# Aster32/GAN-DANet

Hardware: AMD Instinct MI355X
Metric: train samples/sec (G+D step) on 256x256 tiles (higher is better)
Workload: dtype bf16; 1 GPU; full G+D train step, 8ch 256x256 -> 1024x1024 tiles, batch 32/GPU (global 32), perceptual=on, SSIM evaluated, AdamW x2; survey_config=3, per_gpu_batch=32, global_batch=32, tile=256, parallelism=dp1

## Files before the change

### gan-danet_amd/_lib.py

```python
from __future__ import annotations

import ctypes as C
import os

HERE = os.path.dirname(os.path.abspath(__file__))
LIB_PATH = os.path.join(HERE, "lib", "libgandanet_hip.so")

PREC_FP32, PREC_BF16, PREC_X3 = 0, 1, 2
PAM_BWD_K64_ATOMIC, PAM_BWD_K64_PARTS, PAM_BWD_K32_PARTS, PAM_BWD_TWO_KERNEL = 0, 1, 2, 3
ACT_NONE, ACT_RELU, ACT_LEAKY02, ACT_SIGMOID = 0, 1, 2, 3
EVAL_F64, EVAL_SKIP_NAN = 1, 2
GUARD_SQNORM, GUARD_NORM, GUARD_COEF, GUARD_OK, GUARD_APPLIED, GUARD_SKIPPED, GUARD_RECORD = range(7)
GUARD_CHUNK = 65536
FILTER_F32, FILTER_F64 = 0, 1
EDGE_REFLECT, EDGE_INTERIOR = 0, 1
FILTER_MAX_RADIUS, SAVGOL_MAX_WINDOW = 64, 33
ZOOM_MIRROR, ZOOM_NEAREST = 0, 1
FREQ_MAX_BINS, FREQ_MAX_TABLE_BYTES = 33, 16 << 20
ZONE_MAX, ZONE_EDGE_CHUNK = 32, 512
STL_MAX_T = 2048
SKILL_MAPS = ("n", "mean_p", "mean_t", "bias", "rmse", "mae", "std_p", "std_t", "cc", "nse", "kge", "crmsd")
LSTSQ_MAX_P = 8
TREND_MAX_T = 2048
TREND_MAPS = ("n", "s", "var_s", "z", "p", "tau", "slope", "intercept", "slope_lo", "slope_hi")
# ... 5 lines not shown
ENSV_M_COVER, ENSV_M_RELIABILITY, ENSV_M_TIED, ENSV_M_HIST, ENSV_METRICS = 6, 10, 11, 12, 45
ENSV_LEVELS = (0.5, 0.6826894921370859, 0.9, 0.95)
EOF_MAX_T, EOF_MAX_K = 256, 16
EOF_CHUNK, EOF_SPLIT_MIN, EOF_SPLIT_MAX = 32, 8, 256

c_fp = C.c_void_p


class ConvDesc(C.Structure):
    _fields_ = [
        ("B", C.c_int), ("M", C.c_int), ("Mstore", C.c_int), ("Ck", C.c_int), ("ks", C.c_int),
        ("stride", C.c_int), ("pad", C.c_int), ("transposed", C.c_int),
        ("Hi", C.c_int), ("Wi", C.c_int), ("Ho", C.c_int), ("Wo", C.c_int),
        ("a", c_fp), ("a_bs", C.c_long), ("a_sm", C.c_long), ("a_sc", C.c_long), ("a_st", C.c_long),
        ("x", c_fp), ("x_bs", C.c_long),
        ("in_scale", c_fp), ("in_shift", c_fp), ("in_relu", C.c_int),
        ("y", c_fp), ("y_bs", C.c_long),
        ("out_layout", C.c_int), ("out_bf16", C.c_int), ("ldo", C.c_int),
        ("alpha", c_fp), ("bias", c_fp), ("res", c_fp), ("res_bs", C.c_long),
        ("act", C.c_int), ("accumulate", C.c_int), ("precision", C.c_int),
        ("sub_oy", C.c_int), ("sub_ox", C.c_int), ("sub_step", C.c_int),
    ]


class GemmNTDesc(C.Structure):
    _fields_ = [
        ("B", C.c_int), ("M", C.c_int), ("N", C.c_int), ("kseg", C.c_int), ("klen", C.c_long),
        ("a", c_fp), ("a_bs", C.c_long), ("a_ss", C.c_long), ("lda", C.c_long),
        ("bm", c_fp), ("b_bs", C.c_long), ("b_ss", C.c_long), ("ldb", C.c_long),
        ("im2col", C.c_int), ("ks", C.c_int), ("stride", C.c_int), ("pad", C.c_int),
        ("Hi", C.c_int), ("Wi", C.c_int), ("Ho", C.c_int), ("Wo", C.c_int),
        ("in_scale", c_fp), ("in_shift", c_fp), ("in_relu", C.c_int),
        ("c", c_fp), ("c_bs", C.c_long), ("ldc", C.c_long),
        ("alpha", c_fp), ("bias", c_fp),
        ("accumulate", C.c_int), ("splits", C.c_int), ("precision", C.c_int),
    ]


_i, _l, _f, _p, _sz = C.c_int, C.c_long, C.c_float, c_fp, C.c_size_t

SIGNATURES = {
    "gd_version": (_i, []),
    "gd_set_deterministic": (None, [_i]),
    "gd_get_deterministic": (_i, []),
    "gd_set_det_reduce": (_i, [_i]),
    "gd_get_det_reduce": (_i, []),
    "gd_last_error": (_i, [C.c_char_p, _i]),
    "gd_sizeof_conv_desc": (_i, []),
    "gd_sizeof_gemm_nt_desc": (_i, []),
    "gd_conv2d": (_i, [C.POINTER(ConvDesc), _p]),
    "gd_gemm_nt": (_i, [C.POINTER(GemmNTDesc), _p]),
    "gd_gemm_nt_ws": (_i, [C.POINTER(GemmNTDesc), _p, _p, _sz]),
    "gd_gemm_nt_plan": (_i, [C.POINTER(GemmNTDesc), _sz, C.POINTER(_i), C.POINTER(_sz)]),
    "gd_conv3x3_ws_bytes": (_sz, [_i, _i]),
    "gd_conv3x3_eligible": (_i, [C.POINTER(ConvDesc)]),
    "gd_conv3x3": (_i, [C.POINTER(ConvDesc), _p, _sz, _p]),
    "gd_conv3x3_wgrad": (_i, [_p, _l, _p, _p, _l, _p, _i, _p, _p, _i, _i, _i, _i, _i, _i, _i, _i, _p, _p]),
    "gd_conv3x3_wgrad_ws": (_i, [_p, _l, _p, _p, _l, _p, _i, _p, _p, _i, _i, _i, _i, _i, _i, _i, _i, _p, _p, _p, _sz]),
    "gd_conv3x3_wgrad_plan": (_i, [_i, _i, _i, _i, _i, _i, _sz, C.POINTER(_i), C.POINTER(_sz)]),
    "gd_pack_16_split": (_i, [_p, _l, _i, _i, _i, _p, _p, _i, _p, _l, _i, _l, _i, _i, _p, _l, _i, _l, _i, _i, _p]),
    "gd_pack_16_split_masked": (_i, [_p, _l, _i, _i, _i, _p, _p, _i, _p, _l, _i, _l, _i, _i, _p, _l, _i, _l, _i, _i, _p, _l, _p]),
    "gd_split3_weights": (_i, [_p, _l, _l, _l, _p, _p]),
    "gd_bn_stats_ws_floats": (_sz, [_i, _i, _l]),
    "gd_bn_stats": (_i, [_p, _l, _i, _i, _l, _f, _f, _p, _p, _p, _p, _p, _p]),
    "gd_bn_fold": (_i, [_p, _p, _p, _p, _i, _p, _p, _p]),
    "gd_bn_fold_eval": (_i, [_p, _p, _p, _p, _f, _i, _p, _p, _p, _p]),
    "gd_affine_act": (_i, [_p, _l, _p, _p, _i, _i, _l, _i, _p, _l, _p]),
    "gd_bn_act_bwd": (_i, [_p, _l, _p, _l, _p, _p, _p, _p, _p, _i, _i, _l, _i, _i, _p, _p, _p, _l, _i, _p, _p]),
    "gd_bn_stats_local": (_i, [_p, _l, _i, _i, _l, _p, _p, _p]),
    "gd_bn_stats_merge": (_i, [_p, _i, _i, _f, _f, _p, _p, _p, _p, _p]),
    "gd_bn_act_bwd_dx": (_i, [_p, _l, _p, _l, _p, _p, _p, _p, _p, _p, _f, _i, _i, _l, _i, _p, _l, _i, _p]),
    "gd_bicubic_fwd": (_i, [_p, _i, _i, _i, _p, _i, _i, _f, _f, _p]),
    "gd_bicubic_bwd": (_i, [_p, _i, _i, _i, _p, _i, _i, _f, _f, _p]),
    "gd_bilinear_fwd": (_i, [_p, _i, _i, _i, _p, _i, _i, _i, _p, _p]),
    "gd_bilinear_bwd": (_i, [_p, _i, _i, _i, _p, _i, _i, _p]),
    "gd_maxpool2_fwd": (_i, [_p, _i, _i, _i, _p, _p]),
    "gd_maxpool2_bwd": (_i, [_p, _p, _i, _i, _i, _p, _p]),
    "gd_act_fwd": (_i, [_p, _p, _l, _i, _p]),
    "gd_act_bwd": (_i, [_p, _p, _p, _l, _i, _p]),
    "gd_axpby": (_i, [_p, _f, _p, _f, _l, _p]),
    "gd_scale_dev": (_i, [_p, _p, _p, _l, _i, _p]),
    "gd_copy_rows": (_i, [_p, _l, _l, _p, _l, _l, _i, _i, _i, _p]),
    "gd_channel_sum": (_i, [_p, _l, _i, _i, _l, _p, _i, _p, _p]),
    "gd_copy_slab": (_i, [_p, _l, _p, _l, _i, _l, _i, _p]),
    "gd_softmax_rows": (_i, [_p, _p, _l, _i, _f, _p]),
    "gd_softmax_rows_bwd": (_i, [_p, _p, _p, _l, _i, _f, _p]),
    "gd_dot": (_i, [_p, _p, _l, _p, _i, _p, _p]),
    "gd_transpose": (_i, [_p, _p, _i, _i, _i, _p]),
    "gd_add_transpose": (_i, [_p, _p, _i, _i, _p]),
    "gd_bce_logits": (_i, [_p, _l, _f, _p, _p, _p, _p]),
    "gd_bce_logits_target": (_i, [_p, _p, _l, _p, _p, _p, _p, _p]),
    "gd_leaky_fwd": (_i, [_p, _p, _l, _f, _p]),
    "gd_leaky_bwd": (_i, [_p, _p, _p, _l, _f, _p]),
    "gd_mse": (_i, [_p, _p, _l, _p, _p, _p, _p]),
    "gd_l1": (_i, [_p, _p, _l, _p, _p, _p, _p]),
    "gd_tv": (_i, [_p, _i, _i, _i, _i, _f, _p, _p, _p, _p]),
    "gd_ssim": (_i, [_p, _p, _i, _i, _i, _i, _p, _p, _p]),
    "gd_ssim_samples": (_i, [_p, _p, _i, _i, _i, _i, _i, _p, _p, _p]),
    "gd_ssim_bwd": (_i, [_p, _p, _p, _i, _i, _i, _i, _i, _p, _p, _p, _p]),
    "gd_adamw": (_i, [_p, _p, _p, _p, _l, _i, _f, _f, _f, _f, _f, _f, _p]),
    "gd_pam_flash_fwd": (_i, [_p, _p, _p, _i, _i, _i, _i, _i, _i, _i, _p, _p, _l, _p, _l, _p, _p, _p, _p]),
    "gd_pam_key_sqnorm_max": (_i, [_p, _i, _i, _i, _i, _p, _p]),
    "gd_pam_fwd_shift_ws_bytes": (_sz, [_i, _i]),
    "gd_pam_flash_fwd_shift": (_i, [_p, _p, _p, _i, _i, _i, _i, _i, _i, _p, _p, _l, _p, _l, _p, _p, _i, _p, _sz, _p]),
    "gd_pam_flash_bwd": (_i, [_p, _p, _p, _p, _p, _p, _p, _i, _i, _i, _i, _i, _i, _p, _p, _p, _l, _p, _sz, _p]),
    "gd_pam_bwd_scratch_bytes": (_sz, [_i, _i]),
# ... 149 lines not shown
```

### gan-danet_amd/build.py

```python
from __future__ import annotations

import os
import subprocess
import sys
from concurrent.futures import ThreadPoolExecutor

HERE = os.path.dirname(os.path.abspath(__file__))
CSRC = os.path.join(HERE, "csrc")
OUT_DIR = os.path.join(HERE, "lib")
LIB = os.path.join(OUT_DIR, "libgandanet_hip.so")
SOURCES = ["api.hip", "gemm_conv.hip", "conv3x3.hip", "gemm_nt.hip", "norm.hip", "resample.hip", "pointwise.hip", "nhwc.hip", "disc_nhwc.hip", "pam.hip", "pam_bwd64.hip", "pam_wide.hip", "pam_f32.hip", "comm.hip", "histmatch.hip", "det_reduce.hip", "evalstats.hip", "gradguard.hip", "filters.hip", "spline.hip", "prepare.hip", "basins.hip", "stl.hip", "series.hip", "trend.hip", "ensverify.hip", "eof.hip", "pam_probe.hip"]
FLAGS = ["--offload-arch=gfx950", "-O3", "-fPIC", "-std=c++17", "-fno-gpu-rdc", "-Wall", "-Wno-unused-function"]


def _stale(target: str, deps) -> bool:
    if not os.path.exists(target):
        return True
    t = os.path.getmtime(target)
    return any(os.path.getmtime(d) > t for d in deps)


def build(force: bool = False, verbose: bool = True) -> str:
    hipcc = os.environ.get("HIPCC", "/opt/rocm/bin/hipcc")
    os.makedirs(OUT_DIR, exist_ok=True)
    headers = [os.path.join(CSRC, f) for f in os.listdir(CSRC) if f.endswith(".h")]
    headers.append(os.path.join(HERE, "..", "include", "gandanet.h"))
    objs, jobs = [], []
    for src in SOURCES:
        s = os.path.join(CSRC, src)
        o = os.path.join(OUT_DIR, src.replace(".hip", ".o"))
        objs.append(o)
        if force or _stale(o, [s] + headers):
            jobs.append([hipcc, *FLAGS, "-c", s, "-o", o])

    def run(cmd):
        if verbose:
            print(" ".join(cmd), flush=True)
        r = subprocess.run(cmd, capture_output=True, text=True)
        if r.returncode != 0:
            raise RuntimeError(f"hipcc failed:\n{' '.join(cmd)}\n{r.stdout}\n{r.stderr}")
        return r

    with ThreadPoolExecutor(max_workers=4) as ex:
        list(ex.map(run, jobs))
    if force or jobs or _stale(LIB, objs):
        run([hipcc, "--offload-arch=gfx950", "-shared", "-fPIC", "-o", LIB, *objs, "-ldl"])
    return LIB


if __name__ == "__main__":
    print(build(force="--force" in sys.argv))
```

### gan-danet_amd/kern.py

```python
from __future__ import annotations

import ctypes as C
import math
import os
from typing import Optional, Tuple

import torch

from . import _lib as L

Tensor = torch.Tensor


def _stream() -> int:
    return torch.cuda.current_stream().cuda_stream


def _ptr(t: Optional[Tensor]):
    return None if t is None else t.data_ptr()


def _chk(t: Tensor, name: str = "tensor", dtype=torch.float32) -> None:
    if not t.is_cuda:
        raise L.GandanetError(f"{name}: expected a GPU tensor (there is no CPU fallback in the product path)")
# ... 119 lines not shown
    _dense(w, "conv weight")
    B, Cin, Hi, Wi = x.shape
    Cout, Cin_w, k, k2 = w.shape
    if Cin_w != Cin or k != k2:
        raise L.GandanetError(f"conv2d: weight {tuple(w.shape)} does not match input {tuple(x.shape)}")
    Ho, Wo = conv_out_size(Hi, k, stride, pad), conv_out_size(Wi, k, stride, pad)
    if out is None:
        out = torch.empty(B, Cout, Ho, Wo, device=x.device, dtype=torch.float32)
    elif tuple(out.shape) != (B, Cout, Ho, Wo):
        raise L.GandanetError("conv2d: bad out shape")
    with _ConvBracket("fwd", k, stride, Cin, Cout, Ho, Wo, B):
        conv_nn(B=B, M=Cout, Ck=Cin, ks=k, stride=stride, pad=pad, transposed=False, Hi=Hi, Wi=Wi, Ho=Ho, Wo=Wo,
                a=w, a_bs=0, a_sm=Cin * k * k, a_sc=k * k, a_st=1, x=x, x_bs=xbs, y=out, y_bs=_bview(out, "conv out"),
                precision=precision, in_scale=in_scale, in_shift=in_shift, in_relu=in_relu, bias=bias, act=act,
                accumulate=accumulate)
    return out


def conv2d_dgrad(dy: Tensor, w: Tensor, in_hw: Tuple[int, int], stride: int, pad: int, precision: int, *,
                 out: Optional[Tensor] = None, accumulate: bool = False, alpha: Optional[Tensor] = None) -> Tensor:
    dbs = _bview(dy, "conv dy")
    B, Cout, Ho, Wo = dy.shape
    Cout_w, Cin, k, _ = w.shape
    Hi, Wi = in_hw
    if Cout_w != Cout:
        raise L.GandanetError("conv2d_dgrad: weight/out-channel mismatch")
    if out is None:
        out = torch.empty(B, Cin, Hi, Wi, device=dy.device, dtype=torch.float32)
    with _ConvBracket("dgrad", k, stride, Cin, Cout, Ho, Wo, B):
        conv_nn(B=B, M=Cin, Ck=Cout, ks=k, stride=stride, pad=pad, transposed=True, Hi=Ho, Wi=Wo, Ho=Hi, Wo=Wi,
                a=w, a_bs=0, a_sm=k * k, a_sc=Cin * k * k, a_st=1, x=dy, x_bs=dbs, y=out, y_bs=_bview(out, "conv dx"),
                precision=precision, accumulate=accumulate, alpha=alpha)
    return out


def gemm_nt(*, B: int, M: int, N: int, kseg: int, klen: int, a: Tensor, a_bs: int, a_ss: int, lda: int,
            bm: Tensor, b_bs: int, b_ss: int, ldb: int, c: Tensor, c_bs: int, ldc: int, precision: int,
            im2col=None, in_scale=None, in_shift=None, in_relu=False, alpha=None, bias=None,
            accumulate: bool = False, splits: int = 0) -> None:
    d = L.GemmNTDesc()
    d.B, d.M, d.N, d.kseg, d.klen = B, M, N, kseg, klen
    d.a, d.a_bs, d.a_ss, d.lda = _ptr(a), a_bs, a_ss, lda
    d.bm, d.b_bs, d.b_ss, d.ldb = _ptr(bm), b_bs, b_ss, ldb
    if im2col is not None:
        d.im2col = 1
        d.ks, d.stride, d.pad, d.Hi, d.Wi, d.Ho, d.Wo = im2col
    d.in_scale, d.in_shift, d.in_relu = _ptr(in_scale), _ptr(in_shift), int(in_relu)
    d.c, d.c_bs, d.ldc = _ptr(c), c_bs, ldc
    d.alpha, d.bias = _ptr(alpha), _ptr(bias)
    d.accumulate, d.splits, d.precision = int(accumulate), splits, precision
    L.check(lib().gd_gemm_nt_ws(C.byref(d), _stream(), *det_ws()), "gd_gemm_nt")


def conv2d_wgrad(dy: Tensor, x: Tensor, k: int, stride: int, pad: int, precision: int, *, in_scale=None,
                 in_shift=None, in_relu=False, alpha: Optional[Tensor] = None, splits: int = 0) -> Tensor:
    if alpha is not None and not (k == 1 and stride == 1 and pad == 0):
        raise L.GandanetError("conv2d_wgrad: alpha is supported for 1x1 convs only")
    dbs, xbs = _bview(dy, "wgrad dy"), _bview(x, "wgrad x")
    B, Cout, Ho, Wo = dy.shape
    _, Cin, Hi, Wi = x.shape
    dw = torch.empty(Cout, Cin, k, k, device=dy.device, dtype=torch.float32)
    with _ConvBracket("wgrad", k, stride, Cin, Cout, Ho, Wo, B):
        return _conv2d_wgrad(dy, x, k, stride, pad, precision, in_scale, in_shift, in_relu, dw, dbs, xbs, B, Cout, Cin, Hi,
                             Wi, Ho, Wo, alpha, splits)


def _conv2d_wgrad(dy, x, k, stride, pad, precision, in_scale, in_shift, in_relu, dw, dbs, xbs, B, Cout, Cin, Hi, Wi, Ho, Wo,
                  alpha=None, splits=0):
    if USE_CONV3X3_FAST and k == 3 and stride in (1, 2) and pad == 1 and precision == L.PREC_BF16:
        dy16 = x16 = None
        x_ld = 0
        if Cout > 32 and Cin >= 4 * 32:
            dy16, _ = pack_bf16(dy.view(B, Cout, Ho * Wo), Cout, Ho * Wo, plain_shape=(Cout, Ho * Wo))
            if in_scale is None and x.dim() == 4:
                x_ld = (Cin + 7) // 8 * 8
                _, x16 = pack_bf16(x, Cin, Hi * Wi, t_shape=(Hi * Wi, x_ld))
        L.check(lib().gd_conv3x3_wgrad_ws(_ptr(dy), dbs, _ptr(dy16), _ptr(x), xbs, _ptr(x16), x_ld, _ptr(in_scale),
                                       _ptr(in_shift), int(in_relu), B, Cout, Cin, Hi, Wi, stride, 0, _ptr(dw), _stream(),
                                          *det_ws()), "gd_conv3x3_wgrad")
        return dw
    if k == 1 and stride == 1 and pad == 0:
        gemm_nt(B=1, M=Cout, N=Cin, kseg=B, klen=Ho * Wo, a=dy, a_bs=0, a_ss=dbs, lda=Ho * Wo, bm=x, b_bs=0, b_ss=xbs,
                ldb=Hi * Wi, c=dw, c_bs=0, ldc=Cin, precision=precision, in_scale=in_scale, in_shift=in_shift,
                in_relu=in_relu, alpha=alpha, splits=splits)
        return dw
    gemm_nt(B=1, M=Cout, N=Cin * k * k, kseg=B, klen=Ho * Wo, a=dy, a_bs=0, a_ss=dbs, lda=Ho * Wo, bm=x, b_bs=0,
            b_ss=xbs, ldb=0, c=dw, c_bs=0, ldc=Cin * k * k, precision=precision,
            im2col=(k, stride, pad, Hi, Wi, Ho, Wo), in_scale=in_scale, in_shift=in_shift, in_relu=in_relu)
    return dw


def bn_ws(B: int, Cn: int, HW: int, device) -> Tensor:
    n = lib().gd_bn_stats_ws_floats(B, Cn, HW)
    return torch.empty(max(int(n), 1), device=device, dtype=torch.float32)


def channel_sum(x: Tensor, out: Optional[Tensor] = None, accumulate: bool = False) -> Tensor:
    bs = _bview(x, "channel_sum input")
    B, Cn = x.shape[0], x.shape[1]
    HW = x[0, 0].numel()
    if out is None:
        out = torch.empty(Cn, device=x.device, dtype=torch.float32)
    L.check(lib().gd_channel_sum(_ptr(x), bs, B, Cn, HW, _ptr(out), int(accumulate), _ptr(bn_ws(B, Cn, HW, x.device)),
                                 _stream()), "gd_channel_sum")
    return out

# ... 519 lines not shown
    return None


PAM_SCRATCH_CAP = 40 << 30
DETERMINISTIC = False
DET_REDUCE = "unsplit"
_DET_REDUCE_MODES = {"unsplit": 0, "ordered": 1}
DET_WS_BYTES: Optional[int] = None
_DET_WS: dict = {}


def set_deterministic(on: bool, reduce: Optional[str] = None) -> None:
    global DETERMINISTIC, DET_REDUCE
    if reduce is not None and reduce not in _DET_REDUCE_MODES:
        raise L.GandanetError(f"set_deterministic: reduce must be one of {sorted(_DET_REDUCE_MODES)}, got {reduce!r}")
    DETERMINISTIC = bool(on)
    lib().gd_set_deterministic(int(DETERMINISTIC))
    if reduce is not None:
        L.check(lib().gd_set_det_reduce(_DET_REDUCE_MODES[reduce]), "gd_set_det_reduce")
        DET_REDUCE = reduce


def det_ws_bytes() -> int:
    return int(DET_WS_BYTES) if DET_WS_BYTES is not None else int(os.environ.get("GD_DET_WS_MB", "256")) << 20


def det_ws() -> Tuple[Optional[int], int]:
    if not (DETERMINISTIC and DET_REDUCE == "ordered"):
        return None, 0
    nbytes = det_ws_bytes()
    if nbytes <= 0:
        return None, 0
    key = (torch.cuda.current_device(), _stream())
    t = _DET_WS.get(key)
    if t is None or t.numel() != nbytes:
        t = _DET_WS[key] = torch.empty(nbytes, device=torch.device("cuda", key[0]), dtype=torch.uint8)
    return t.data_ptr(), nbytes


def conv3x3_wgrad_plan(B: int, Cout: int, Cin: int, H: int, W: int, stride: int = 1, ws_bytes: Optional[int] = None):
    sp, need = C.c_int(0), C.c_size_t(0)
    nb = det_ws_bytes() if ws_bytes is None else ws_bytes
    L.check(lib().gd_conv3x3_wgrad_plan(B, Cout, Cin, H, W, stride, nb, C.byref(sp), C.byref(need)), "gd_conv3x3_wgrad_plan")
    return sp.value, need.value


def gemm_nt_plan(*, B: int, M: int, N: int, kseg: int, klen: int, splits: int = 0, precision: int = L.PREC_FP32,
                 ws_bytes: Optional[int] = None):
    d = L.GemmNTDesc()
    d.B, d.M, d.N, d.kseg, d.klen, d.splits, d.precision = B, M, N, kseg, klen, splits, precision
    sp, need = C.c_int(0), C.c_size_t(0)
    nb = det_ws_bytes() if ws_bytes is None else ws_bytes
    L.check(lib().gd_gemm_nt_plan(C.byref(d), nb, C.byref(sp), C.byref(need)), "gd_gemm_nt_plan")
    return sp.value, need.value


def pam_bwd_form() -> int:
    return L.PAM_BWD_K64_PARTS if DETERMINISTIC else L.PAM_BWD_K64_ATOMIC


def pam_flash_bwd(qt, kt, kn, vt, dot_, lse, delta, B, N, Npad, Cp, dqn, dkn, dv, r_alg: int = 32, c_alg: int = 0,
                  f16: bool = False, form: Optional[int] = None, out_bs: int = 0):
    form = pam_bwd_form() if form is None else form
    scratch, scratch_bytes = None, 0
    per_image = int(lib().gd_pam_bwd_scratch_bytes(Npad, form))
    if per_image:
        nslices = -(-(B * per_image) // PAM_SCRATCH_CAP)
        images = max(1, -(-B // nslices))
        scratch_bytes = per_image * images
        scratch = torch.empty(scratch_bytes, device=dqn.device, dtype=torch.uint8)
    with _Bracket("pam_flash_bwd", 4.0 * N * N * (r_alg + (c_alg or Cp)) * B):
        L.check(lib().gd_pam_flash_bwd(_ptr(qt), _ptr(kt), _ptr(kn), _ptr(vt), _ptr(dot_), _ptr(lse), _ptr(delta), B,
                                       N, Npad, Cp, int(f16), int(form), _ptr(dqn), _ptr(dkn), _ptr(dv), int(out_bs),
                                       _ptr(scratch), scratch_bytes, _stream()), "gd_pam_flash_bwd")


def pam_wide_slots(r: int) -> int:
    return 32 if r <= 31 else 64


def pam_wide_fwd(qt, kt, v, B, N, Npad, Cn, Cp, D, gamma, x, out, o_attn, lse, r_alg: int, f16: bool = False):
    with _Bracket("pam_wide_fwd", 2.0 * N * N * (r_alg + Cn) * B):
        L.check(lib().gd_pam_wide_fwd(_ptr(qt), _ptr(kt), _ptr(v), B, N, Npad, Cn, Cp, D, int(f16), _ptr(gamma), _ptr(x),
                                      _bview(x), _ptr(out), _bview(out), _ptr(o_attn), _ptr(lse), _stream()),
                "gd_pam_wide_fwd")


def pam_wide_bwd(qt, kt, kn, vt, dot_, lse, delta, B, N, Npad, Cp, D, dqn, dkn, dv, r_alg: int, c_alg: int,
                 f16: bool = False, deterministic: Optional[bool] = None):
    det = DETERMINISTIC if deterministic is None else bool(deterministic)
    scratch, scratch_bytes = None, 0
    per_image = int(lib().gd_pam_wide_scratch_bytes(Npad, D, int(det)))
    if per_image:
        nslices = -(-(B * per_image) // PAM_SCRATCH_CAP)
        scratch_bytes = per_image * max(1, -(-B // nslices))
        scratch = torch.empty(scratch_bytes, device=dqn.device, dtype=torch.uint8)
    with _Bracket("pam_wide_bwd", 4.0 * N * N * (r_alg + c_alg) * B):
        L.check(lib().gd_pam_wide_bwd(_ptr(qt), _ptr(kt), _ptr(kn), _ptr(vt), _ptr(dot_), _ptr(lse), _ptr(delta), B, N,
                                      Npad, Cp, D, int(f16), int(det), _ptr(dqn), _ptr(dkn), _ptr(dv), _ptr(scratch),
                                      scratch_bytes, _stream()), "gd_pam_wide_bwd")


_f32_flash = os.environ.get("GD_PAM_F32_FLASH", "")
PAM_F32_FLASH: Optional[bool] = True if _f32_flash == "1" else False if _f32_flash == "0" else None
PAM_F32_AUTO_ELEMS = 1 << 31

# ... 1185 lines not shown
```

### gan-danet_amd/ops.py

```python
from __future__ import annotations

from typing import List, Optional

import torch
from torch.autograd import Function

from . import _lib as L
from . import kern as K
from .config import config, operand_mode, sixteen_bit

ACT_NONE, ACT_RELU, ACT_LEAKY, ACT_SIGMOID = L.ACT_NONE, L.ACT_RELU, L.ACT_LEAKY02, L.ACT_SIGMOID


def _prec(layer: str = "other") -> int:
    mode = operand_mode(layer)
    return L.PREC_BF16 if mode == "16" else L.PREC_X3 if mode == "x3" else L.PREC_FP32


def _x3(layer: str) -> bool:
    return operand_mode(layer) == "x3"


def _x3_eligible(x, w, stride, pad, act) -> bool:
    return (x.dim() == 4 and tuple(w.shape[2:]) == (3, 3) and stride == 1 and pad == 1 and act in (ACT_NONE, ACT_RELU)
# ... 489 lines not shown
        _, dot_ = K.pack_bf16(d_pam, Cn, N, scale=s_up, t_shape=(Np, Cp), f16=f16)
        if route == "wide":
            D = qt.shape[2]
            dqn = torch.empty(B, D, Np, device=x.device, dtype=torch.float32)
            dkn = torch.empty(B, D, Np, device=x.device, dtype=torch.float32)
            dvp = torch.empty(B, Cp, Np, device=x.device, dtype=torch.float32)
            K.pam_wide_bwd(qt, kt, kn, vt, dot_, lse, delta, B, N, Np, Cp, D, dqn, dkn, dvp, r_alg=r, c_alg=Cn, f16=f16)
        elif Np == N and K.pam_bwd_form() == L.PAM_BWD_K64_ATOMIC:
            R = 64 + Cp
            dcat = torch.empty(B, R, Np, device=x.device, dtype=torch.float32)
            K.pam_flash_bwd(qt, kt, kn, vt, dot_, lse, delta, B, N, Np, Cp, dcat[:, 0:32], dcat[:, 32:64], dcat[:, 64:],
                            r_alg=r, c_alg=Cn, f16=f16, out_bs=R * Np)
            wcat = torch.zeros(R, Cn, 1, 1, device=x.device, dtype=torch.float32)
            for w_, lo in ((wq, 0), (wk, 32), (wv, 64)):
                K.copy_slab(_c(w_).view(1, w_.shape[0], Cn), wcat.view(1, R, Cn)[:, lo:lo + w_.shape[0]])
            dcat4 = dcat.view(B, R, H, W)
            dwc = K.conv2d_wgrad(dcat4, x, 1, 1, 0, prec, alpha=s_inv)
            dbc = K.channel_sum(dcat4) if any(has_bias) else None
            if dbc is not None and s_inv is not None:
                K.scale_dev(dbc, s_inv, out=dbc)
            K.conv2d_dgrad(dcat4, wcat, (H, W), 1, 0, prec, out=dx.view(B, Cn, H, W), accumulate=True, alpha=s_inv)
            grads = []
            for (lo, n), hb in zip(((0, r), (32, r), (64, Cn)), has_bias):
                grads.append(dwc[lo:lo + n])
                grads.append(dbc[lo:lo + n] if hb else None)
            return (*grads, dgamma_p)
        else:
            dqn = torch.empty(B, 32, Np, device=x.device, dtype=torch.float32)
            dkn = torch.empty(B, 32, Np, device=x.device, dtype=torch.float32)
            dvp = torch.empty(B, Cp, Np, device=x.device, dtype=torch.float32)
            K.pam_flash_bwd(qt, kt, kn, vt, dot_, lse, delta, B, N, Np, Cp, dqn, dkn, dvp, r_alg=r, c_alg=Cn, f16=f16)
        if s_inv is not None:
            for t in (dqn, dkn, dvp):
                K.scale_dev(t, s_inv, out=t)
        dq, dk, dv = _compact(dqn, r, N), _compact(dkn, r, N), _compact(dvp, Cn, N)
    else:
        pprec = prec if sixteen_bit("pam") else L.PREC_FP32
        dq, dk, dv, dgamma_p = _pam_chain_bwd(pam_saved, gamma_p, d_pam, pprec)
    grads = []
    splits = 1 if route == "f32" else 0
    for dy3, w, hb in ((dq, wq, has_bias[0]), (dk, wk, has_bias[1]), (dv, wv, has_bias[2])):
        dy4 = dy3.view(B, dy3.shape[1], H, W)
        grads.append(K.conv2d_wgrad(dy4, x, 1, 1, 0, prec, splits=splits))
        grads.append(K.channel_sum(dy4) if hb else None)
        K.conv2d_dgrad(dy4, w, (H, W), 1, 0, prec, out=dx.view(B, Cn, H, W), accumulate=True)
    return (*grads, dgamma_p)


def _cam_forward(x, gamma_c, out3, prec=L.PREC_FP32):
    B, Cn, H, W = x.shape
    N = H * W
    x3 = x.view(B, Cn, N)
    e = torch.empty(B, Cn, Cn, device=x.device, dtype=torch.float32)
    K.gemm_nt(B=B, M=Cn, N=Cn, kseg=1, klen=N, a=x3, a_bs=Cn * N, a_ss=0, lda=N, bm=x3, b_bs=Cn * N, b_ss=0,
              ldb=N, c=e, c_bs=Cn * Cn, ldc=Cn, precision=L.PREC_FP32)
    att = K.softmax_rows(e, -1.0, out=e)
    K.conv_nn(B=B, M=Cn, Ck=Cn, ks=1, stride=1, pad=0, transposed=False, Hi=1, Wi=N, Ho=1, Wo=N, a=att,
              a_bs=Cn * Cn, a_sm=Cn, a_sc=1, a_st=0, x=x3, x_bs=Cn * N, y=out3, y_bs=K._bview(out3),
              precision=prec, alpha=gamma_c, res=x3, res_bs=Cn * N)
    return att


def _cam_backward(att, x, gamma_c, d_cam, dx, prec=L.PREC_FP32):
    B, Cn, H, W = x.shape
    N = H * W
    x3 = x.view(B, Cn, N)
    d_bs = K._bview(d_cam)
    da = torch.empty(B, Cn, Cn, device=x.device, dtype=torch.float32)
    K.gemm_nt(B=B, M=Cn, N=Cn, kseg=1, klen=N, a=d_cam, a_bs=d_bs, a_ss=0, lda=N, bm=x3, b_bs=Cn * N, b_ss=0,
              ldb=N, c=da, c_bs=Cn * Cn, ldc=Cn, precision=L.PREC_FP32)
    dgamma_c = K.dot(att, da)
    de = K.softmax_rows_bwd(att, da, -1.0)
    sym = K.add_transpose(de)
    K.conv_nn(B=B, M=Cn, Ck=Cn, ks=1, stride=1, pad=0, transposed=False, Hi=1, Wi=N, Ho=1, Wo=N, a=att,
              a_bs=Cn * Cn, a_sm=1, a_sc=Cn, a_st=0, x=d_cam, x_bs=d_bs, y=dx, y_bs=Cn * N,
              precision=prec, alpha=gamma_c, accumulate=True)
    K.conv_nn(B=B, M=Cn, Ck=Cn, ks=1, stride=1, pad=0, transposed=False, Hi=1, Wi=N, Ho=1, Wo=N, a=sym,
              a_bs=Cn * Cn, a_sm=Cn, a_sc=1, a_st=0, x=x3, x_bs=Cn * N, y=dx, y_bs=Cn * N,
              precision=prec, alpha=gamma_c, accumulate=True)
    return dgamma_c


class PamFn(Function):

    @staticmethod
    def forward(ctx, x, wq, bq, wk, bk, wv, bv, gamma_p):
        x = _c(x)
        prec = _prec("conv1x1")
        out = torch.empty_like(x)
        route, saved = _pam_forward(x, wq, bq, wk, bk, wv, bv, gamma_p, _as3(out), prec)
        ctx.save_for_backward(x, wq, wk, wv, gamma_p, *saved)
        ctx.cfg = (prec, route, (bq is not None, bk is not None, bv is not None))
        return out

    @staticmethod
    def backward(ctx, dout):
        x, wq, wk, wv, gamma_p, *saved = ctx.saved_tensors
        prec, route, has_bias = ctx.cfg
        B, Cn, H, W = x.shape
        d3 = _as3(_c(dout))
        dx = torch.empty(B, Cn, H * W, device=x.device, dtype=torch.float32)
        K.copy_slab(d3, dx)
        dwq, dbq, dwk, dbk, dwv, dbv, dg = _pam_backward(route, saved, x, wq, wk, wv, gamma_p, d3, dx, prec, has_bias)
        return dx.view(B, Cn, H, W), dwq, dbq, dwk, dbk, dwv, dbv, dg


class CamFn(Function):

    @staticmethod
    def forward(ctx, x, gamma_c):
        x = _c(x)
        out = torch.empty_like(x)
        ctx.prec = _prec("cam_apply")
        att = _cam_forward(x, gamma_c, _as3(out), ctx.prec)
        ctx.save_for_backward(x, gamma_c, att)
        return out

    @staticmethod
    def backward(ctx, dout):
        x, gamma_c, att = ctx.saved_tensors
        B, Cn, H, W = x.shape
        d3 = _as3(_c(dout))
        dx = torch.empty(B, Cn, H * W, device=x.device, dtype=torch.float32)
# ... 507 lines not shown
```

### include/gandanet.h

```cpp
#ifndef GANDANET_H
#define GANDANET_H
#include <stddef.h>
#include <stdint.h>
#ifdef __cplusplus
extern "C" {
#endif

#define GD_VERSION 100
void gd_set_deterministic(int on);
int gd_get_deterministic(void);
int gd_set_det_reduce(int mode);
int gd_get_det_reduce(void);
int gd_version(void);
int gd_last_error(char* buf, int n);
int gd_sizeof_conv_desc(void);
int gd_sizeof_gemm_nt_desc(void);

enum { GD_PREC_FP32 = 0,
       GD_PREC_BF16 = 1,
       GD_PREC_X3 = 2     };
enum { GD_ACT_NONE = 0, GD_ACT_RELU = 1, GD_ACT_LEAKY02 = 2, GD_ACT_SIGMOID = 3 };

typedef struct gd_conv_desc {
    int B;
    int M;
    int Mstore;
    int Ck;
    int ks;
    int stride, pad;
    int transposed;
    int Hi, Wi;
    int Ho, Wo;
    const float* a; long a_bs, a_sm, a_sc, a_st;
    const float* x; long x_bs;
    const float* in_scale; const float* in_shift; int in_relu;
    void* y; long y_bs;
    int out_layout;
    int out_bf16;
    int ldo;
    const float* alpha; const float* bias; const float* res; long res_bs;
    int act; int accumulate;
    int precision;
    int sub_oy, sub_ox, sub_step;
} gd_conv_desc;
int gd_conv2d(const gd_conv_desc* d, void* stream);

size_t gd_conv3x3_ws_bytes(int M, int Ck);
int gd_conv3x3_eligible(const gd_conv_desc* d);
int gd_conv3x3(const gd_conv_desc* d, void* ws, size_t ws_bytes, void* stream);
int gd_conv3x3_wgrad(const float* dy, long dy_bs, const void* dy_bf16, const float* x, long x_bs, const void* x_nhwc16,
                     int x_ld, const float* in_scale, const float* in_shift, int in_relu, int B, int Cout, int Cin, int H,
                     int W, int stride, int accumulate, float* dw, void* stream);
int gd_conv3x3_wgrad_ws(const float* dy, long dy_bs, const void* dy_bf16, const float* x, long x_bs, const void* x_nhwc16,
                        int x_ld, const float* in_scale, const float* in_shift, int in_relu, int B, int Cout, int Cin, int H,
                        int W, int stride, int accumulate, float* dw, void* stream, void* ws, size_t ws_bytes);
int gd_conv3x3_wgrad_plan(int B, int Cout, int Cin, int H, int W, int stride, size_t ws_bytes, int* splits, size_t* ws_needed);

typedef struct gd_gemm_nt_desc {
    int B, M, N;
    int kseg; long klen;
    const float* a; long a_bs, a_ss, lda;
    const float* bm; long b_bs, b_ss, ldb;
    int im2col, ks, stride, pad, Hi, Wi, Ho, Wo;
    const float* in_scale; const float* in_shift; int in_relu;
    float* c; long c_bs, ldc;
    const float* alpha;
    const float* bias;
    int accumulate;
    int splits;
    int precision;
} gd_gemm_nt_desc;
int gd_gemm_nt(const gd_gemm_nt_desc* d, void* stream);
int gd_gemm_nt_ws(const gd_gemm_nt_desc* d, void* stream, void* ws, size_t ws_bytes);
int gd_gemm_nt_plan(const gd_gemm_nt_desc* d, size_t ws_bytes, int* splits, size_t* ws_needed);

size_t gd_bn_stats_ws_floats(int B, int C, long HW);
int gd_bn_stats(const float* x, long x_bs, int B, int C, long HW, float eps, float momentum,
                float* mean, float* invstd, float* running_mean, float* running_var, float* ws, void* stream);
int gd_bn_fold(const float* gamma, const float* beta, const float* mean, const float* invstd, int C,
               float* scale, float* shift, void* stream);
int gd_bn_stats_local(const float* x, long x_bs, int B, int C, long HW, float* stats, float* ws, void* stream);
int gd_bn_stats_merge(const float* stats_all, int world, int C, float eps, float momentum, float* mean, float* invstd,
                      float* running_mean, float* running_var, void* stream);
int gd_bn_act_bwd_dx(const float* dy, long dy_bs, const float* x, long x_bs, const float* scale, const float* shift,
                     const float* mean, const float* invstd, const float* dgamma_sum, const float* dbeta_sum, float inv_n,
                     int B, int C, long HW, int act, float* dx, long dx_bs, int accumulate_dx, void* stream);
int gd_bn_fold_eval(const float* gamma, const float* beta, const float* running_mean, const float* running_var,
                    float eps, int C, float* scale, float* shift, float* invstd_out, void* stream);
int gd_channel_sum(const float* x, long x_bs, int B, int C, long HW, float* out, int accumulate, float* ws,
                   void* stream);
int gd_affine_act(const float* x, long x_bs, const float* scale, const float* shift, int B, int C, long HW,
                  int act, float* y, long y_bs, void* stream);
int gd_bn_act_bwd(const float* dy, long dy_bs, const float* x, long x_bs, const float* scale, const float* shift,
                  const float* mean, const float* invstd, const float* gamma, int B, int C, long HW, int act,
                  int train, float* dgamma, float* dbeta, float* dx, long dx_bs, int accumulate_dx, float* ws,
                  void* stream);

int gd_bicubic_fwd(const float* x, int BC, int Hi, int Wi, float* y, int Ho, int Wo, float rscale_h,
                   float rscale_w, void* stream);
int gd_bicubic_bwd(const float* dy, int BC, int Hi, int Wi, float* dx, int Ho, int Wo, float rscale_h,
                   float rscale_w, void* stream);
int gd_shift_sum9_fwd(const float* u, const float* bias, float* y, int B, int H, int W, void* stream);
int gd_shift_sum9_bwd(const float* dy, float* du, int B, int H, int W, void* stream);
int gd_combine_inputs(const float* lr, int C1, int H1, int W1, float rs1, const float* aux, int C2, int H2, int W2,
                      float rs2, float* out, int B, int Ho, int Wo, void* stream);
int gd_bilinear_fwd(const float* x, int BC, int Hi, int Wi, float* y, int Ho, int Wo, int accumulate,
                    const float* res, void* stream);
int gd_bilinear_bwd(const float* dy, int BC, int Hi, int Wi, float* dx, int Ho, int Wo, void* stream);
int gd_maxpool2_fwd(const float* x, int BC, int Hi, int Wi, float* y, void* stream);
int gd_maxpool2_bwd(const float* x, const float* dy, int BC, int Hi, int Wi, float* dx, void* stream);

int gd_act_fwd(const float* x, float* y, long n, int act, void* stream);
int gd_act_bwd(const float* y, const float* dy, float* dx, long n, int act, void* stream);
int gd_axpby(const float* x, float a, float* y, float b, long n, void* stream);
int gd_scale_dev(const float* x, const float* s_dev, float* y, long n, int accumulate, void* stream);
int gd_copy_rows(const float* src, long s_bs, long s_ld, float* dst, long d_bs, long d_ld, int B, int R, int Cc,
                 void* stream);
int gd_copy_slab(const float* src, long s_bs, float* dst, long d_bs, int B, long chw, int accumulate, void* stream);
int gd_softmax_rows(const float* x, float* y, long rows, int cols, float sign, void* stream);
int gd_softmax_rows_bwd(const float* p, const float* dp, float* dx, long rows, int cols, float sign, void* stream);
int gd_dot(const float* a, const float* b, long n, float* out, int accumulate, float* ws, void* stream);
int gd_transpose(const float* s, float* t, int B, int R, int Cc, void* stream);
int gd_add_transpose(const float* a, float* out, int B, int n, void* stream);

int gd_bce_logits(const float* z, long n, float label, float* out, float* dz, float* ws, void* stream);
int gd_bce_logits_target(const float* z, const float* t, long n, float* out, float* dz, float* dt, float* ws,
                         void* stream);
// ... 266 lines not shown
```

Before: 38.31 samples/s.

## Add dedicated CAM Gram kernel with whole-matrix block tiles and symmetric reuse

Adds a specialised fp32 MFMA kernel for the channel-attention Gram products (C x C from C x N operands, C up to 192). Each block computes the whole output matrix, with split-K across blocks and wave-assigned 32x32 tiles. When both operands are the same tensor it computes only the upper triangle, loads one shared tile, and mirrors the result. It targets the CAM forward energy and backward gradient GEMMs, which have small M and N but long K and likely map poorly onto the generic gemm_nt. The cost is a new code path plus extra zero and mirror launches, and atomic split-K reductions when not in deterministic mode.

New measurement: 38.57 samples/s (median of 6 runs). About the same (+0.7%).

```diff
diff --git a/gan-danet_amd/_lib.py b/gan-danet_amd/_lib.py
--- a/gan-danet_amd/_lib.py
+++ b/gan-danet_amd/_lib.py
@@ -81,6 +81,9 @@
     "gd_gemm_nt": (_i, [C.POINTER(GemmNTDesc), _p]),
     "gd_gemm_nt_ws": (_i, [C.POINTER(GemmNTDesc), _p, _p, _sz]),
     "gd_gemm_nt_plan": (_i, [C.POINTER(GemmNTDesc), _sz, C.POINTER(_i), C.POINTER(_sz)]),
+    "gd_cam_gram_eligible": (_i, [C.POINTER(GemmNTDesc)]),
+    "gd_cam_gram_ws": (_i, [C.POINTER(GemmNTDesc), _p, _p, _sz]),
+    "gd_cam_gram_plan": (_i, [C.POINTER(GemmNTDesc), _sz, C.POINTER(_i), C.POINTER(_sz)]),
     "gd_conv3x3_ws_bytes": (_sz, [_i, _i]),
     "gd_conv3x3_eligible": (_i, [C.POINTER(ConvDesc)]),
     "gd_conv3x3": (_i, [C.POINTER(ConvDesc), _p, _sz, _p]),
diff --git a/gan-danet_amd/build.py b/gan-danet_amd/build.py
--- a/gan-danet_amd/build.py
+++ b/gan-danet_amd/build.py
@@ -9,7 +9,7 @@
 CSRC = os.path.join(HERE, "csrc")
 OUT_DIR = os.path.join(HERE, "lib")
 LIB = os.path.join(OUT_DIR, "libgandanet_hip.so")
-SOURCES = ["api.hip", "gemm_conv.hip", "conv3x3.hip", "gemm_nt.hip", "norm.hip", "resample.hip", "pointwise.hip", "nhwc.hip", "disc_nhwc.hip", "pam.hip", "pam_bwd64.hip", "pam_wide.hip", "pam_f32.hip", "comm.hip", "histmatch.hip", "det_reduce.hip", "evalstats.hip", "gradguard.hip", "filters.hip", "spline.hip", "prepare.hip", "basins.hip", "stl.hip", "series.hip", "trend.hip", "ensverify.hip", "eof.hip", "pam_probe.hip"]
+SOURCES = ["api.hip", "gemm_conv.hip", "conv3x3.hip", "gemm_nt.hip", "cam_gram.hip", "norm.hip", "resample.hip", "pointwise.hip", "nhwc.hip", "disc_nhwc.hip", "pam.hip", "pam_bwd64.hip", "pam_wide.hip", "pam_f32.hip", "comm.hip", "histmatch.hip", "det_reduce.hip", "evalstats.hip", "gradguard.hip", "filters.hip", "spline.hip", "prepare.hip", "basins.hip", "stl.hip", "series.hip", "trend.hip", "ensverify.hip", "eof.hip", "pam_probe.hip"]
 FLAGS = ["--offload-arch=gfx950", "-O3", "-fPIC", "-std=c++17", "-fno-gpu-rdc", "-Wall", "-Wno-unused-function"]
 
 
diff --git a/gan-danet_amd/csrc/cam_gram.hip b/gan-danet_amd/csrc/cam_gram.hip
--- /dev/null
+++ b/gan-danet_amd/csrc/cam_gram.hip
@@ -0,0 +1,337 @@
+#include <type_traits>
+
+#include "common.h"
+#include "tile_mma.h"
+#include "../../include/gandanet.h"
+
+namespace {
+
+constexpr int BK = gd::TILE_BK;
+constexpr int LD = gd::TilePol<gd::MODE_F32>::LD;
+constexpr int WMAX = 192;
+constexpr int NT = WMAX / 32;
+constexpr int RG = WMAX / 32;
+constexpr int MAX_TILES = 9;
+
+template <int I, int N, class F>
+__device__ __forceinline__ void static_for(F&& f) {
+    if constexpr (I < N) {
+        f(std::integral_constant<int, I>{});
+        static_for<I + 1, N>(f);
+    }
+}
+
+template <bool SYM>
+constexpr int tile_owner(int tm, int tn) {
+    if constexpr (SYM) {
+        if (tn < tm) return -1;
+        if (tn < NT - 1) return (tm * (NT - 1) - tm * (tm - 1) / 2 + (tn - tm)) % 4;
+        constexpr int last[NT] = {3, 3, 0, 1, 2, 0};
+        return last[tm];
+    } else {
+        if (tm < NT - 1 && tn < NT - 1) return (tm * (NT - 1) + tn) % 4;
+        const int e = tm == NT - 1 ? tn : NT + tm;
+        return e < 9 ? 1 + e % 3 : 0;
+    }
+}
+
+struct TileList {
+    int n;
+    int tm[MAX_TILES], tn[MAX_TILES];
+    unsigned rows, cols;
+};
+
+template <bool SYM>
+constexpr TileList make_list(int w, int nt) {
+    TileList l{};
+    for (int tm = 0; tm < nt; ++tm)
+        for (int tn = 0; tn < nt; ++tn)
+            if (tile_owner<SYM>(tm, tn) == w) {
+                l.tm[l.n] = tm;
+                l.tn[l.n] = tn;
+                l.rows |= 1u << tm;
+                l.cols |= 1u << tn;
+                ++l.n;
+            }
+    return l;
+}
+constexpr bool lists_fit() {
+    for (int w = 0; w < 4; ++w)
+        if (make_list<true>(w, NT).n > MAX_TILES || make_list<false>(w, NT).n > MAX_TILES) return false;
+    int total = 0, total_sym = 0;
+    for (int w = 0; w < 4; ++w) {
+        total += make_list<false>(w, NT).n;
+        total_sym += make_list<true>(w, NT).n;
+    }
+    return total == NT * NT && total_sym == NT * (NT + 1) / 2;
+}
+static_assert(lists_fit(), "every tile needs exactly one wave, and a wave at most nine tiles");
+
+__global__ void gram_zero_kernel(float* c, long c_bs, long ldc, int B, int M, int N) {
+    const long total = (long)B * M * N;
+    for (long i = (long)blockIdx.x * blockDim.x + threadIdx.x; i < total; i += (long)gridDim.x * blockDim.x) {
+        const int n = (int)(i % N);
+        const long t = i / N;
+        c[(t / M) * c_bs + (t % M) * ldc + n] = 0.f;
+    }
+}
+
+__global__ void gram_mirror_kernel(float* c, long c_bs, long ldc, int B, int M) {
+    const long total = (long)B * M * M;
+    for (long i = (long)blockIdx.x * blockDim.x + threadIdx.x; i < total; i += (long)gridDim.x * blockDim.x) {
+        const int n = (int)(i % M);
+        const long t = i / M;
+        const int m = (int)(t % M);
+        float* cb = c + (t / M) * c_bs;
+        if (n < m) cb[(long)m * ldc + n] = cb[(long)n * ldc + m];
+    }
+}
+
+struct GramArgs {
+    const float* a; long a_bs, lda;
+    const float* b; long b_bs, ldb;
+    float* c; long c_bs, ldc;
+    const float* alpha;
+    float* part;
+    int B, M, N;
+    long klen;
+    int ktiles, tiles_per_split, splits, accumulate;
+};
+
+template <bool SYM, int NTL, int W>
+__device__ __forceinline__ void gram_wave(const GramArgs& g, float* As, float* Bs, int tid, int b, int split) {
+    constexpr TileList TL = make_list<SYM>(W, NTL ? NTL : NT);
+    constexpr bool MASKED = NTL == 0;
+    const int lane = tid & 63;
+    const int r = lane & 31, h = lane >> 5;
+    const int kq = tid & 7, r0v = tid >> 3;
+
+    unsigned live = 0;
+#pragma unroll
+    for (int i = 0; i < TL.n; ++i)
+        if (TL.tm[i] * 32 < g.M && TL.tn[i] * 32 < g.N) live |= 1u << i;
+
+    f32x16_t acc[TL.n > 0 ? TL.n : 1];
+#pragma unroll
+    for (int i = 0; i < TL.n; ++i)
+#pragma unroll
+        for (int e = 0; e < 16; ++e) acc[i][e] = 0.f;
+
+    const float* a_base = g.a + (long)b * g.a_bs;
+    const float* b_base = g.b + (long)b * g.b_bs;
+    const int ga = (g.M + 31) >> 5, gb = (g.N + 31) >> 5;
+    const unsigned off_a = r0v * (unsigned)g.lda + kq * 4, off_b = r0v * (unsigned)g.ldb + kq * 4;
+    float4 va[RG], vb[SYM ? 1 : RG];
+
+    auto load_tile = [&](int t) {
+        const long k = (long)t * BK + kq * 4;
+        const bool k_ok = k < g.klen;
+        const float* ap = a_base + (long)t * BK;
+        const float* bp = b_base + (long)t * BK;
+#pragma unroll
+        for (int i = 0; i < RG; ++i) {
+            if (i >= ga) break;
+            const int m = r0v + 32 * i;
+            va[i] = (k_ok && m < g.M) ? *reinterpret_cast<const float4*>(ap + (long)(32 * i) * g.lda + off_a) : make_float4(0, 0, 0, 0);
+        }
+        if constexpr (!SYM) {
+#pragma unroll
+            for (int i = 0; i < RG; ++i) {
+                if (i >= gb) break;
+                const int n = r0v + 32 * i;
+                vb[i] = (k_ok && n < g.N) ? *reinterpret_cast<const float4*>(bp + (long)(32 * i) * g.ldb + off_b) : make_float4(0, 0, 0, 0);
+            }
+        }
+    };
+    auto store_tile = [&]() {
+#pragma unroll
+        for (int i = 0; i < RG; ++i) {
+            if (i >= ga) break;
+            float* p = As + (r0v + 32 * i) * LD + kq * 4;
+            p[0] = va[i].x; p[1] = va[i].y; p[2] = va[i].z; p[3] = va[i].w;
+        }
+        if constexpr (!SYM) {
+#pragma unroll
+            for (int i = 0; i < RG; ++i) {
+                if (i >= gb) break;
+                float* p = Bs + (r0v + 32 * i) * LD + kq * 4;
+                p[0] = vb[i].x; p[1] = vb[i].y; p[2] = vb[i].z; p[3] = vb[i].w;
+            }
+        }
+    };
+
+    const int t_begin = split * g.tiles_per_split;
+    const int t_end = min(g.ktiles, t_begin + g.tiles_per_split);
+
+    load_tile(t_begin);
+    store_tile();
+    __syncthreads();
+    for (int t = t_begin; t < t_end; ++t) {
+        if (t + 1 < t_end) load_tile(t + 1);
+#pragma unroll 2
+        for (int ks = 0; ks < BK / 2; ++ks) {
+            float fa[NT], fb[NT];
+            static_for<0, NT>([&](auto tc) {
+                constexpr int T = decltype(tc)::value;
+                constexpr TileList L = make_list<SYM>(W, NTL ? NTL : NT);
+                constexpr bool in_a = (L.rows >> T) & 1, in_b = (L.cols >> T) & 1;
+                if constexpr (in_a) fa[T] = As[(T * 32 + r) * LD + ks * 2 + h];
+                if constexpr (in_b) {
+                    if constexpr (SYM && in_a) fb[T] = fa[T];
+                    else fb[T] = Bs[(T * 32 + r) * LD + ks * 2 + h];
+                }
+            });
+            static_for<0, TL.n>([&](auto ic) {
+                constexpr int I = decltype(ic)::value;
+                constexpr TileList L = make_list<SYM>(W, NTL ? NTL : NT);
+                if (!MASKED || ((live >> I) & 1))
+                    acc[I] = __builtin_amdgcn_mfma_f32_32x32x2f32(fa[L.tm[I]], fb[L.tn[I]], acc[I], 0, 0, 0);
+            });
+        }
+        __syncthreads();
+        if (t + 1 < t_end) {
+            store_tile();
+            __syncthreads();
+        }
+    }
+
+    const float alpha = g.alpha ? *g.alpha : 1.f;
+    const bool atomic = !g.part && g.splits > 1;
+    float* cb = g.part ? g.part + ((long)split * g.B + b) * g.M * g.N : g.c + (long)b * g.c_bs;
+    const long ld = g.part ? g.N : g.ldc;
+    static_for<0, TL.n>([&](auto ic) {
+        constexpr int I = decltype(ic)::value;
+        constexpr TileList L = make_list<SYM>(W, NTL ? NTL : NT);
+        if (!((live >> I) & 1)) return;
+        const int n = L.tn[I] * 32 + r;
+        if (n >= g.N) return;
+#pragma unroll
+        for (int e = 0; e < 16; ++e) {
+            const int m = L.tm[I] * 32 + gd::acc_row(e, h);
+            if (m >= g.M) continue;
+            const float v = acc[I][e] * alpha;
+            float* cp = cb + (long)m * ld + n;
+            if constexpr (SYM) {
+                if (n < m) continue;
+                if (atomic) {
+                    atomicAdd(cp, v);
+                } else {
+                    *cp = v;
+                    if (n > m) cb[(long)n * ld + m] = v;
+                }
+            } else {
+                if (atomic) atomicAdd(cp, v);
+                else if (g.accumulate && !g.part) *cp += v;
+                else *cp = v;
+            }
+        }
+    });
+}
+
+template <bool SYM, int NTL>
+__global__ __launch_bounds__(256, 2) void cam_gram_kernel(const GramArgs g) {
+    __shared__ __attribute__((aligned(16))) float S[(SYM ? 1 : 2) * WMAX * LD];
+    float* As = S;
+    float* Bs = SYM ? S : S + WMAX * LD;
+    const int tid = threadIdx.x;
+    const int b = blockIdx.x / g.splits;
+    const int split = blockIdx.x - b * g.splits;
+    for (int i = tid; i < (SYM ? 1 : 2) * WMAX * LD; i += 256) S[i] = 0.f;
+    __syncthreads();
+    switch (__builtin_amdgcn_readfirstlane(tid >> 6)) {
+        case 0: gram_wave<SYM, NTL, 0>(g, As, Bs, tid, b, split); break;
+        case 1: gram_wave<SYM, NTL, 1>(g, As, Bs, tid, b, split); break;
+        case 2: gram_wave<SYM, NTL, 2>(g, As, Bs, tid, b, split); break;
+        default: gram_wave<SYM, NTL, 3>(g, As, Bs, tid, b, split); break;
+    }
+}
+
+bool gram_served(const gd_gemm_nt_desc& d) {
+    return d.B > 0 && d.M > 0 && d.N > 0 && d.M <= WMAX && d.N <= WMAX && d.kseg == 1 && d.klen > 0 &&
+           d.klen < (1L << 31) && d.lda < (1L << 24) && d.ldb < (1L << 24) && !d.im2col && !d.in_scale && !d.in_shift && !d.bias && d.precision == GD_PREC_FP32 &&
+           d.klen % 4 == 0 && d.lda % 4 == 0 && d.ldb % 4 == 0 && d.a_bs % 4 == 0 && d.b_bs % 4 == 0 &&
+           ((uintptr_t)d.a % 16) == 0 && ((uintptr_t)d.bm % 16) == 0;
+}
+
+struct GramPlan { int ktiles, tiles_per_split, splits, ordered; size_t ws_needed; };
+int gram_plan(const gd_gemm_nt_desc& d, size_t ws_bytes, GramPlan* p) {
+    GD_CHECK_ARG(d.B > 0 && d.M > 0 && d.N > 0 && d.klen > 0, "gd_cam_gram: bad sizes");
+    GD_CHECK_ARG(d.M <= WMAX && d.N <= WMAX, "gd_cam_gram: serves M, N <= 192 only");
+    GD_CHECK_ARG(gram_served(d), "gd_cam_gram: descriptor not served (fp32, one segment, plain operands, 16-byte rows)");
+    const int ktiles = gd_cdiv(d.klen, BK);
+    int splits = d.splits;
+    if (splits <= 0) {
+        splits = 512 / d.B;
+        if (splits < 1) splits = 1;
+        if (splits > ktiles / 8) splits = ktiles / 8 > 0 ? ktiles / 8 : 1;
+    }
+    if (splits > ktiles) splits = ktiles;
+    const bool det = gd_get_deterministic() != 0, ordered_mode = det && gd_get_det_reduce() == 1;
+    if (det && !ordered_mode) splits = 1;
+    const size_t out_bytes = (size_t)d.B * d.M * d.N * sizeof(float);
+    if (ordered_mode) {
+        const size_t fit = ws_bytes / out_bytes;
+        if ((size_t)splits > fit) splits = (int)fit;
+        if (splits < 2) splits = 1;
+    }
+    const int tps = (ktiles + splits - 1) / splits;
+    splits = (ktiles + tps - 1) / tps;
+    GD_CHECK_ARG((long)d.B * splits < (1L << 31), "gd_cam_gram: batch too large");
+    p->ktiles = ktiles; p->tiles_per_split = tps; p->splits = splits;
+    p->ordered = ordered_mode && splits > 1;
+    p->ws_needed = p->ordered ? (size_t)splits * out_bytes : 0;
+    return 0;
+}
+
+template <bool SYM>
+void launch_gram(const GramArgs& g, hipStream_t s) {
+    const dim3 grid((unsigned)(g.B * g.splits));
+    const int nt = max(gd_cdiv(g.M, 32), gd_cdiv(g.N, 32));
+    const bool square = gd_cdiv(g.M, 32) == gd_cdiv(g.N, 32);
+    if (square && nt == 6) hipLaunchKernelGGL((cam_gram_kernel<SYM, 6>), grid, dim3(256), 0, s, g);
+    else if (square && nt == 5) hipLaunchKernelGGL((cam_gram_kernel<SYM, 5>), grid, dim3(256), 0, s, g);
+    else hipLaunchKernelGGL((cam_gram_kernel<SYM, 0>), grid, dim3(256), 0, s, g);
+}
+
+}
+
+extern "C" int gd_cam_gram_eligible(const gd_gemm_nt_desc* d) { return d != nullptr && gram_served(*d); }
+
+extern "C" int gd_cam_gram_plan(const gd_gemm_nt_desc* dp, size_t ws_bytes, int* splits, size_t* ws_needed) {
+    GD_CHECK_ARG(dp != nullptr, "gd_cam_gram_plan: null descriptor");
+    GramPlan p;
+    if (gram_plan(*dp, ws_bytes, &p)) return -1;
+    if (splits) *splits = p.splits;
+    if (ws_needed) *ws_needed = p.ws_needed;
+    return 0;
+}
+
+extern "C" int gd_cam_gram_ws(const gd_gemm_nt_desc* dp, void* stream, void* ws, size_t ws_bytes) {
+    GD_CHECK_ARG(dp != nullptr, "gd_cam_gram: null descriptor");
+    const gd_gemm_nt_desc& d = *dp;
+    GD_CHECK_ARG(d.a && d.bm && d.c, "gd_cam_gram: null tensor");
+    GD_CHECK_ARG(((uintptr_t)ws % 16) == 0, "gd_cam_gram: the workspace must be 16-byte aligned");
+    GramPlan p;
+    if (gram_plan(d, ws ? ws_bytes : 0, &p)) return -1;
+    hipStream_t s = (hipStream_t)stream;
+    const bool sym = d.a == d.bm && d.a_bs == d.b_bs && d.lda == d.ldb && d.M == d.N && !d.accumulate;
+    GramArgs g;
+    g.a = d.a; g.a_bs = d.a_bs; g.lda = d.lda;
+    g.b = d.bm; g.b_bs = d.b_bs; g.ldb = d.ldb;
+    g.c = d.c; g.c_bs = d.c_bs; g.ldc = d.ldc;
+    g.alpha = d.alpha;
+    g.part = p.ordered ? (float*)ws : nullptr;
+    g.B = d.B; g.M = d.M; g.N = d.N; g.klen = d.klen;
+    g.ktiles = p.ktiles; g.tiles_per_split = p.tiles_per_split; g.splits = p.splits; g.accumulate = d.accumulate;
+    const bool atomic = p.splits > 1 && !g.part;
+    const long total = (long)d.B * d.M * d.N;
+    const int blocks = (int)((total + 255) / 256 > 4096 ? 4096 : (total + 255) / 256);
+    if (atomic && !d.accumulate)
+        hipLaunchKernelGGL(gram_zero_kernel, dim3(blocks), dim3(256), 0, s, d.c, d.c_bs, d.ldc, d.B, d.M, d.N);
+    if (sym) launch_gram<true>(g, s);
+    else launch_gram<false>(g, s);
+    if (sym && atomic) hipLaunchKernelGGL(gram_mirror_kernel, dim3(blocks), dim3(256), 0, s, d.c, d.c_bs, d.ldc, d.B, d.M);
+    GD_LAUNCH_CHECK();
+    if (g.part) return gd_det_reduce_launch(g.part, p.splits, d.c, d.B, d.M, d.N, d.c_bs, d.ldc, nullptr, d.accumulate, s);
+    return 0;
+}
diff --git a/gan-danet_amd/kern.py b/gan-danet_amd/kern.py
--- a/gan-danet_amd/kern.py
+++ b/gan-danet_amd/kern.py
@@ -195,6 +195,38 @@
     L.check(lib().gd_gemm_nt_ws(C.byref(d), _stream(), *det_ws()), "gd_gemm_nt")
 
 
+def _gram_desc(B, M, N, klen, a, a_bs, lda, bm, b_bs, ldb, c, c_bs, ldc, alpha, accumulate, splits):
+    d = L.GemmNTDesc()
+    d.B, d.M, d.N, d.kseg, d.klen = B, M, N, 1, klen
+    d.a, d.a_bs, d.lda = _ptr(a), a_bs, lda
+    d.bm, d.b_bs, d.ldb = _ptr(bm), b_bs, ldb
+    d.c, d.c_bs, d.ldc = _ptr(c), c_bs, ldc
+    d.alpha = _ptr(alpha)
+    d.accumulate, d.splits, d.precision = int(accumulate), splits, L.PREC_FP32
+    return d
+
+
+def cam_gram_eligible(*, B: int, M: int, N: int, klen: int, a: Optional[Tensor] = None, a_bs: int = 0, lda: int = 0,
+                      bm: Optional[Tensor] = None, b_bs: int = 0, ldb: int = 0) -> bool:
+    d = _gram_desc(B, M, N, klen, a, a_bs, lda, bm, b_bs, ldb, None, 0, 0, None, False, 0)
+    return bool(lib().gd_cam_gram_eligible(C.byref(d)))
+
+
+def cam_gram(*, B: int, M: int, N: int, klen: int, a: Tensor, a_bs: int, lda: int, bm: Tensor, b_bs: int, ldb: int,
+             c: Tensor, c_bs: int, ldc: int, alpha=None, accumulate: bool = False, splits: int = 0) -> None:
+    d = _gram_desc(B, M, N, klen, a, a_bs, lda, bm, b_bs, ldb, c, c_bs, ldc, alpha, accumulate, splits)
+    L.check(lib().gd_cam_gram_ws(C.byref(d), _stream(), *det_ws()), "gd_cam_gram")
+
+
+def gram_nt(*, B: int, M: int, N: int, klen: int, a: Tensor, a_bs: int, lda: int, bm: Tensor, b_bs: int, ldb: int,
+            c: Tensor, c_bs: int, ldc: int) -> None:
+    if cam_gram_eligible(B=B, M=M, N=N, klen=klen, a=a, a_bs=a_bs, lda=lda, bm=bm, b_bs=b_bs, ldb=ldb):
+        cam_gram(B=B, M=M, N=N, klen=klen, a=a, a_bs=a_bs, lda=lda, bm=bm, b_bs=b_bs, ldb=ldb, c=c, c_bs=c_bs, ldc=ldc)
+    else:
+        gemm_nt(B=B, M=M, N=N, kseg=1, klen=klen, a=a, a_bs=a_bs, a_ss=0, lda=lda, bm=bm, b_bs=b_bs, b_ss=0, ldb=ldb,
+                c=c, c_bs=c_bs, ldc=ldc, precision=L.PREC_FP32)
+
+
 def conv2d_wgrad(dy: Tensor, x: Tensor, k: int, stride: int, pad: int, precision: int, *, in_scale=None,
                  in_shift=None, in_relu=False, alpha: Optional[Tensor] = None, splits: int = 0) -> Tensor:
     if alpha is not None and not (k == 1 and stride == 1 and pad == 0):
@@ -820,6 +852,14 @@
     sp, need = C.c_int(0), C.c_size_t(0)
     nb = det_ws_bytes() if ws_bytes is None else ws_bytes
     L.check(lib().gd_gemm_nt_plan(C.byref(d), nb, C.byref(sp), C.byref(need)), "gd_gemm_nt_plan")
+    return sp.value, need.value
+
+
+def cam_gram_plan(*, B: int, M: int, N: int, klen: int, splits: int = 0, ws_bytes: Optional[int] = None):
+    d = _gram_desc(B, M, N, klen, None, M * klen, klen, None, N * klen, klen, None, 0, 0, None, False, splits)
+    sp, need = C.c_int(0), C.c_size_t(0)
+    nb = det_ws_bytes() if ws_bytes is None else ws_bytes
+    L.check(lib().gd_cam_gram_plan(C.byref(d), nb, C.byref(sp), C.byref(need)), "gd_cam_gram_plan")
     return sp.value, need.value
 
 
diff --git a/gan-danet_amd/ops.py b/gan-danet_amd/ops.py
--- a/gan-danet_amd/ops.py
+++ b/gan-danet_amd/ops.py
@@ -565,8 +565,7 @@
     N = H * W
     x3 = x.view(B, Cn, N)
     e = torch.empty(B, Cn, Cn, device=x.device, dtype=torch.float32)
-    K.gemm_nt(B=B, M=Cn, N=Cn, kseg=1, klen=N, a=x3, a_bs=Cn * N, a_ss=0, lda=N, bm=x3, b_bs=Cn * N, b_ss=0,
-              ldb=N, c=e, c_bs=Cn * Cn, ldc=Cn, precision=L.PREC_FP32)
+    K.gram_nt(B=B, M=Cn, N=Cn, klen=N, a=x3, a_bs=Cn * N, lda=N, bm=x3, b_bs=Cn * N, ldb=N, c=e, c_bs=Cn * Cn, ldc=Cn)
     att = K.softmax_rows(e, -1.0, out=e)
     K.conv_nn(B=B, M=Cn, Ck=Cn, ks=1, stride=1, pad=0, transposed=False, Hi=1, Wi=N, Ho=1, Wo=N, a=att,
               a_bs=Cn * Cn, a_sm=Cn, a_sc=1, a_st=0, x=x3, x_bs=Cn * N, y=out3, y_bs=K._bview(out3),
@@ -580,8 +579,7 @@
     x3 = x.view(B, Cn, N)
     d_bs = K._bview(d_cam)
     da = torch.empty(B, Cn, Cn, device=x.device, dtype=torch.float32)
-    K.gemm_nt(B=B, M=Cn, N=Cn, kseg=1, klen=N, a=d_cam, a_bs=d_bs, a_ss=0, lda=N, bm=x3, b_bs=Cn * N, b_ss=0,
-              ldb=N, c=da, c_bs=Cn * Cn, ldc=Cn, precision=L.PREC_FP32)
+    K.gram_nt(B=B, M=Cn, N=Cn, klen=N, a=d_cam, a_bs=d_bs, lda=N, bm=x3, b_bs=Cn * N, ldb=N, c=da, c_bs=Cn * Cn, ldc=Cn)
     dgamma_c = K.dot(att, da)
     de = K.softmax_rows_bwd(att, da, -1.0)
     sym = K.add_transpose(de)
diff --git a/include/gandanet.h b/include/gandanet.h
--- a/include/gandanet.h
+++ b/include/gandanet.h
@@ -73,6 +73,10 @@
 int gd_gemm_nt(const gd_gemm_nt_desc* d, void* stream);
 int gd_gemm_nt_ws(const gd_gemm_nt_desc* d, void* stream, void* ws, size_t ws_bytes);
 int gd_gemm_nt_plan(const gd_gemm_nt_desc* d, size_t ws_bytes, int* splits, size_t* ws_needed);
+
+int gd_cam_gram_eligible(const gd_gemm_nt_desc* d);
+int gd_cam_gram_ws(const gd_gemm_nt_desc* d, void* stream, void* ws, size_t ws_bytes);
+int gd_cam_gram_plan(const gd_gemm_nt_desc* d, size_t ws_bytes, int* splits, size_t* ws_needed);
 
 size_t gd_bn_stats_ws_floats(int B, int C, long HW);
 int gd_bn_stats(const float* x, long x_bs, int B, int C, long HW, float eps, float momentum,
```
